# HuttleyLab/DiverseSeq

Measured on AMD Instinct MI355X. Metric: sequences scored/sec (delta-JSD, k=6), higher is better.
Workload: dtype f64 (results and every set update in f64; reject/accept decisions tiered: f32 and f32-log scores decide rows farther from the threshold than their proven error bands, f64 the rest)

## Files before the change

### diverseseq_amd/csrc/api.cpp

```cpp
#include "dvs_internal.h"

#include <cmath>
#include <cstring>
#include <mutex>

uint64_t dvs_pow_u64(uint32_t base, uint32_t exp, bool *overflow);
void dvs_matrix_free_fields(dvs_matrix *m);
int dvs_matrix_fill_counts(dvs_ctx *ctx, dvs_matrix *m, const dvs_seq_view &sv, const uint64_t *offsets, bool no_wait);
int dvs_matrix_fill_freq_entropy(dvs_ctx *ctx, dvs_matrix *m);
int dvs_hist_prepare(dvs_ctx *ctx, const uint64_t *offsets, uint32_t nseq, uint32_t k, uint64_t nbins, uint64_t nbytes, size_t *n_long_out);
bool dvs_hist_rows_fit_u16(const dvs_ctx *ctx, uint64_t B, size_t n_long);
int dvs_matrix_fill_freq_totals(dvs_ctx *ctx, dvs_matrix *m, const double *d_meta);
int dvs_matrix_fill_compacted(dvs_ctx *ctx, dvs_matrix *m, const double *d_in, const double *d_meta);

static std::string g_create_err;

int dvs_set_error(dvs_ctx *ctx, int code, const char *fmt, ...) {
    char buf[512];
    va_list ap;
    va_start(ap, fmt);
    vsnprintf(buf, sizeof buf, fmt, ap);
    va_end(ap);
    if (ctx) ctx->err = buf;
    else g_create_err = buf;
// ... 25 lines not shown
    if (e != hipSuccess) {
        *ptr = nullptr;
        return dvs_hip_fail(ctx, e, what);
    }
    ctx->live[*ptr] = sz;
    return DVS_OK;
}

void dvs_dev_free(dvs_ctx *ctx, void *ptr) {
    if (!ptr) return;
    auto it = ctx ? ctx->live.find(ptr) : std::map<void *, size_t>::iterator();
    if (!ctx || it == ctx->live.end()) {
        (void)hipFree(ptr);
        return;
    }
    ctx->pool.emplace(it->second, ptr);
    ctx->pool_bytes += it->second;
    ctx->live.erase(it);
}

int dvs_pinned_get(dvs_ctx *ctx, void **ptr) {
    if (!ctx->pinned_pool.empty()) {
        *ptr = ctx->pinned_pool.back();
        ctx->pinned_pool.pop_back();
        return DVS_OK;
    }
    hipError_t e = hipHostMalloc(ptr, 4096, hipHostMallocDefault);
    if (e != hipSuccess) return dvs_hip_fail(ctx, e, "hipHostMalloc");
    return DVS_OK;
}
void dvs_pinned_put(dvs_ctx *ctx, void *ptr) {
    if (!ptr) return;
    if (ctx) ctx->pinned_pool.push_back(ptr);
    else (void)hipHostFree(ptr);
}
hipEvent_t dvs_event_get(dvs_ctx *ctx) {
    if (!ctx->event_pool.empty()) {
        hipEvent_t e = ctx->event_pool.back();
        ctx->event_pool.pop_back();
        return e;
    }
    hipEvent_t e = nullptr;
    (void)hipEventCreate(&e);
    return e;
}
void dvs_event_put(dvs_ctx *ctx, hipEvent_t e) {
    if (!e) return;
    if (ctx) ctx->event_pool.push_back(e);
    else (void)hipEventDestroy(e);
}

void dvs_dev_trim(dvs_ctx *ctx) {
    (void)hipStreamSynchronize(ctx->stream);
    for (auto &kv : ctx->pool) (void)hipFree(kv.second);
    ctx->pool.clear();
    ctx->pool_bytes = 0;
}

void dvs_knobs_from_env(dvs_knobs *k) {
    auto on = [](const char *name) { return getenv(name) != nullptr; };
    *k = dvs_knobs();
    k->no_uniform_offsets = on("DVS_NO_UNIFORM_OFFSETS");
    k->no_offsets_cache = on("DVS_NO_OFFSETS_CACHE");
    k->counts_u32 = on("DVS_COUNTS_U32");
    k->build_wait = on("DVS_BUILD_WAIT");
    k->no_packed_upload = on("DVS_NO_PACKED_UPLOAD");
// ... 103 lines not shown
    const uint32_t words = uint32_t(ctx->n_cu + 31) / 32;
    std::vector<uint32_t> lo(words, 0u), hi(words, 0u);
    for (int i = 0; i < ctx->n_cu; i++) (i < head ? lo : hi)[i / 32] |= 1u << (i % 32);
    hipStream_t a = nullptr, b = nullptr;
    if (hipExtStreamCreateWithCUMask(&a, words, lo.data()) != hipSuccess ||
        hipExtStreamCreateWithCUMask(&b, words, hi.data()) != hipSuccess) {
        (void)hipGetLastError();
        if (a) (void)hipStreamDestroy(a);
        return false;
    }
    ctx->stream_head = a;
    ctx->stream_rest = b;
    ctx->head_cus = head;
    return true;
}

void dvs_ctx_retain(dvs_ctx *ctx) {
    if (ctx) ctx->refs++;
}

void dvs_ctx_release(dvs_ctx *ctx) {
    if (!ctx || --ctx->refs > 0) return;
    (void)hipSetDevice(ctx->device);
    dvs_dev_free(ctx, ctx->off_cache.d_off);
    dvs_dev_free(ctx, ctx->off_cache.d_rows);
    dvs_dev_free(ctx, ctx->off_cache.d_tiles);
    if (ctx->off_cache.ev_up) (void)hipEventDestroy(ctx->off_cache.ev_up);
    if (ctx->off_cache.h_off) (void)hipHostFree(ctx->off_cache.h_off);
    if (ctx->pack_ev) (void)hipEventDestroy(ctx->pack_ev);
    if (ctx->h_pack) (void)hipHostFree(ctx->h_pack);
    dvs_dev_free(ctx, ctx->d_clog_tbl);
    dvs_dev_trim(ctx);
    for (void *p : ctx->pinned_pool) (void)hipHostFree(p);
    for (hipEvent_t e : ctx->event_pool) (void)hipEventDestroy(e);
    if (ctx->stream2) (void)hipStreamDestroy(ctx->stream2);
    if (ctx->stream_head) (void)hipStreamDestroy(ctx->stream_head);
    if (ctx->stream_rest) (void)hipStreamDestroy(ctx->stream_rest);
    if (ctx->own_stream && ctx->stream) (void)hipStreamDestroy(ctx->stream);
    delete ctx;
}

extern "C" {

const char *dvs_last_error(const dvs_ctx *ctx) { return ctx ? ctx->err.c_str() : g_create_err.c_str(); }

int dvs_ctx_trim(dvs_ctx *ctx) {
    if (!ctx) return DVS_ERR_VALUE;
    dvs_dev_trim(ctx);
    return DVS_OK;
}

int dvs_ctx_sync(dvs_ctx *ctx) {
    if (!ctx) return DVS_ERR_VALUE;
    DVS_HIP(ctx, hipStreamSynchronize(ctx->stream));
    return DVS_OK;
}

int dvs_ctx_set_timing(dvs_ctx *ctx, int on) {
    if (!ctx) return DVS_ERR_VALUE;
    ctx->timing = on != 0;
    return DVS_OK;
}

int dvs_ctx_device_info(dvs_ctx *ctx, char *name, size_t name_len, int *n_cu, uint64_t *hbm_bytes) {
    if (!ctx) return DVS_ERR_VALUE;
    hipDeviceProp_t prop;
// ... 299 lines not shown
```

### diverseseq_amd/csrc/dvs_internal.h

```cpp
#pragma once

#include <hip/hip_runtime.h>

#include <cstdarg>
#include <cstdint>
#include <cstdio>
#include <functional>
#include <map>
#include <string>
#include <vector>

#include "../../include/dvs_hip.h"

#define DVS_EPS 2.220446049250313e-16
#define DVS_HEAD_ROWS 1024u

struct dvs_knobs {
    bool no_uniform_offsets = false;
    bool no_offsets_cache = false;
    bool counts_u32 = false;
    bool build_wait = false;
    bool no_packed_upload = false;
    bool cu_mask_set = false;
    bool no_fast_step = false;
    bool no_persist = false;
    bool no_head_phase = false;
    bool persist_no_seeded = false;
    bool persist_no_small = false;
    bool persist_no_coarse = false;
    bool persist_no_events = false;
    bool persist_debug = false;
    int persist_wg_rounds = -1;
    bool ingest_no_stream = false;
    bool test_persist_fake_error = false;
    uint32_t test_long_tile = 0;
    uint32_t test_rowlog_ring = 0;
};
void dvs_knobs_from_env(dvs_knobs *k);

struct dvs_ctx {
    dvs_knobs knobs;
    int device = 0;
    hipStream_t stream = nullptr;
    bool own_stream = false;
    hipStream_t stream2 = nullptr;
    hipStream_t stream_head = nullptr, stream_rest = nullptr;
    int head_cus = 0;
    bool cu_split_tried = false;
    int persist_timeouts = 0;
    int n_cu = 0;
    size_t lds_per_block = 0;
    double *d_clog_tbl = nullptr;
    bool timing = false;
    std::string err;
    std::multimap<size_t, void *> pool;
    std::vector<void *> pinned_pool;
    std::vector<hipEvent_t> event_pool;
    std::map<void *, size_t> live;
    size_t pool_bytes = 0;
    int refs = 1;
    bool owner_gone = false;
    std::map<const void *, size_t> lds_raised;
    std::map<std::pair<const void *, size_t>, bool> persist_fits;
    struct OffsetsCache {
        uint64_t *h_off = nullptr;
        size_t h_cap = 0, n_off = 0;
        hipEvent_t ev_up = nullptr;
        std::vector<uint32_t> h_long_rows;
        std::vector<unsigned char> h_tiles;
        uint64_t nbytes = 0;
        uint32_t k = 0;
        void *d_off = nullptr, *d_rows = nullptr, *d_tiles = nullptr;
        size_t d_off_cap = 0;
        size_t n_long = 0, n_tiles = 0;
        bool uniform = false;
        uint64_t uni_base = 0, uni_stride = 0;
    } off_cache;
    void *h_pack = nullptr;
    size_t h_pack_cap = 0;
    hipEvent_t pack_ev = nullptr;
};
int dvs_raise_dyn_lds(dvs_ctx *ctx, const void *fn, size_t bytes);
void dvs_ctx_retain(dvs_ctx *ctx);
hipStream_t dvs_ctx_stream2(dvs_ctx *ctx);
bool dvs_ctx_cu_split(dvs_ctx *ctx);
void dvs_ctx_release(dvs_ctx *ctx);

struct dvs_matrix;
int dvs_matrix_settle(dvs_ctx *ctx, const dvs_matrix *m);
int dvs_dev_alloc(dvs_ctx *ctx, void **ptr, size_t bytes, const char *what);
void dvs_dev_free(dvs_ctx *ctx, void *ptr);
void dvs_dev_trim(dvs_ctx *ctx);
struct PooledBuf {
    dvs_ctx *ctx;
    void *p = nullptr;
    ~PooledBuf() { dvs_dev_free(ctx, p); }
    template <typename T>
    T *as() { return static_cast<T *>(p); }
};
int dvs_pinned_get(dvs_ctx *ctx, void **ptr);
void dvs_pinned_put(dvs_ctx *ctx, void *ptr);
hipEvent_t dvs_event_get(dvs_ctx *ctx);
void dvs_event_put(dvs_ctx *ctx, hipEvent_t e);

int dvs_set_error(dvs_ctx *ctx, int code, const char *fmt, ...);
int dvs_hip_fail(dvs_ctx *ctx, hipError_t e, const char *what);

#define DVS_HIP(ctx, call)                                        \
    do {                                                          \
        hipError_t e__ = (call);                                  \
        if (e__ != hipSuccess) return dvs_hip_fail(ctx, e__, #call); \
    } while (0)

struct dvs_matrix {
    int kind = 0;
    uint16_t *d_counts16 = nullptr;
    uint32_t nrows = 0;
    uint64_t nbins = 0;
    uint32_t k = 0, num_states = 0;
    uint32_t *d_counts = nullptr;
    double *d_freqs = nullptr;
    uint32_t *d_totals = nullptr;
    double *d_entropy = nullptr;
    uint32_t *d_src_row = nullptr;
    std::vector<uint32_t> h_head_totals;
    uint32_t *h_head_pinned = nullptr;
    hipEvent_t ev_built = nullptr;
    hipEvent_t ev_join = nullptr;
    uint32_t head_count = 0;
    uint32_t head_rows_built = 0;
    bool rest_beside_head = false;
    int device = 0;
    dvs_ctx *ctx = nullptr;
};
// ... 135 lines not shown
```

### diverseseq_amd/csrc/persist.hip

```cpp
#include "select_dev.h"

#include <algorithm>
#include <type_traits>
#include <cstddef>
#include <cstdlib>
#include <cstring>

namespace {

constexpr int P_THREADS = 512;
constexpr int P_J = 8;
constexpr int P_CH = 16;
constexpr uint32_t P_MAXN = 512;
constexpr uint32_t P_MAXN_BIG = 256;
constexpr uint32_t P_MAXN_MAX = 896;
constexpr uint32_t p_maxn(bool cached, bool maxm = false) { return cached ? (maxm ? P_MAXN_MAX : P_MAXN) : P_MAXN_BIG; }
constexpr uint32_t P_SMALLN = 16;
constexpr uint32_t P_SMALL_ROWS = 13;
constexpr uint32_t p_maxjobs(bool cached, bool maxm = false) { return p_maxn(cached, maxm) + 1; }
constexpr size_t p_acc_bytes(uint32_t maxn) { return size_t(8) * (maxn + 1) * 2 * sizeof(unsigned long long); }
__device__ __forceinline__ unsigned long long p_acc_word(double v) {
    return ((unsigned long long)__double2ll_rn(v * 0x1p50) << 6) + 1ull;
}
__device__ __forceinline__ double p_acc_value(unsigned long long w) { return double((long long)w >> 6) * 0x1p-50; }
// ... 2810 lines not shown
            const unsigned long long d1 = p_acc_complete(acc + uint64_t(tid) * 2 + 1, s_prev + tid * 2 + 1, HO_K, acc_ok);
            unsigned long long e0 = 0ull, e1 = 0ull;
            for (uint32_t q = 0; q < HO_K; q++) {
                const uint32_t h2 = ho_hash(epoch, tid * HO_K + q);
                e0 += p_acc_word(double((h2 >> 4) & 0xFFFFu) * (1.0 / 65536.0));
                e1 += p_acc_word(double(h2 & 0xFFu) * (1.0 / 4096.0));
            }
            acc_wrong = !acc_ok || d0 != e0 || d1 != e1;
        }
        if (__syncthreads_or(acc_wrong ? 1 : 0) && tid == 0) fails++;
        if (mirror && epoch + 1 < rounds) {
            if (tid == 0) __hip_atomic_store(&sync->wrec[(epoch + 1) & 1u][b], p_word(epoch + 1, SEL_NONE, false), RLX_AGENT);
            early_rec = epoch + 1;
            for (uint32_t z = (h >> 16) & 15u; z > 0; z--) __builtin_amdgcn_s_sleep(16);
        }
    }
    if (tid == 0 && fails) atomicAdd(bad, fails);
    if (tid == 0 && __hip_atomic_load(&sync->timeout, RLX_AGENT)) atomicAdd(bad, 1ull << 32);
}

}

template <typename T>
static const void *persist_fn(const dvs_select *s) {
    const bool cached = s->dev.B <= uint64_t(P_J) * P_THREADS;
    if (s->params.mode == DVS_MODE_MAX) return reinterpret_cast<const void *>(persist_nmost_kernel<T, true, true>);
    if constexpr (std::is_same_v<T, uint16_t>) {
        if (s->persist_small) return reinterpret_cast<const void *>(persist_nmost_kernel<T, true, false, true>);
    }
    return cached ? reinterpret_cast<const void *>(persist_nmost_kernel<T, true>)
                  : reinterpret_cast<const void *>(persist_nmost_kernel<T, false>);
}

static int persist_prepare(dvs_ctx *ctx, dvs_select *s, uint32_t head_stop, hipStream_t on) {
    std::vector<unsigned char> &image = head_stop ? s->h_psync_head : s->h_psync;
    image.assign(sizeof(PSync), 0);
    PSync &init = *reinterpret_cast<PSync *>(image.data());
    init.stop_at = head_stop;
    init.seeded = s->persist_seeded ? 1u : 0u;
    init.seed_list = static_cast<const unsigned long long *>(s->d_seed_list);
    for (int g = 0; g < 8; g++) init.rel[g].hint = ~0ull;
    init.wg_thresh = s->params.window ? 0u : 4u;
    init.wg_scale = 1.5f;
    if (ctx->knobs.persist_wg_rounds >= 0) init.wg_thresh = uint32_t(ctx->knobs.persist_wg_rounds);
    init.no_coarse = (ctx->knobs.persist_no_coarse ? 1u : 0u) | (ctx->knobs.persist_no_events ? 2u : 0u) |
                     0u;
    init.small_rows = s->persist_small ? s->persist_small_rows : 0u;
    init.lds_bytes = uint32_t(s->persist_lds);
    init.wmax = uint32_t(std::min<uint64_t>(s->npos, 0xFFFFFFFFull));
    DVS_HIP(ctx, hipMemcpyAsync(head_stop ? s->psync_head : s->psync, &init, sizeof init, hipMemcpyHostToDevice, on));
    DVS_HIP(ctx, hipMemsetAsync(head_stop ? s->ppart_head : s->ppart, 0, p_acc_bytes(s->persist_maxn), on));
    return DVS_OK;
}

template <typename T>
static int persist_launch(dvs_ctx *ctx, dvs_select *s, const T *mat, uint32_t grid, uint32_t head_stop,
                          hipStream_t on) {
    const SelDev &d = s->dev;
    if (head_stop ? !s->head_prepared : !s->persist_prepared) {
        int prc = persist_prepare(ctx, s, head_stop, on);
        if (prc) return prc;
    }
    if (head_stop) s->head_prepared = false;
    else s->persist_prepared = false;
    s->persist_seeded = false;
    const hipEvent_t e1 = dvs_scan_timing_start(ctx, s, on);
    const void *fn = persist_fn<T>(s);
    SelDev d_arg = d;
    const T *mat_arg = mat;
    PSync *sync_arg = static_cast<PSync *>(head_stop ? s->psync_head : s->psync);
    unsigned long long *part_arg = static_cast<unsigned long long *>(head_stop ? s->ppart_head : s->ppart);
    uint32_t g_arg = grid;
    void *args[] = {&d_arg, &mat_arg, &sync_arg, &part_arg, &g_arg};
    hipError_t le = hipLaunchKernel(fn, dim3(grid), dim3(P_THREADS), args, s->persist_lds, on);
    if (s->time_scan) (void)hipEventRecord(e1, on);
    if (le != hipSuccess) {
        (void)hipGetLastError();
        return DVS_ERR_UNSUPPORTED;
    }
    DVS_HIP(ctx, hipGetLastError());
    return DVS_OK;
}

int dvs_persist_setup(dvs_ctx *ctx, dvs_select *s) {
// ... 17 lines not shown
               size_t(maxn_ + 1) * 16 +
               (maxm ? p_batch_lds() : 0);
    };
    size_t lds = lds_for(p_maxn(cached, maxm));
    if (s->persist_small) {
        const size_t lds_small = lds_for(P_SMALLN) + size_t(s->persist_small_rows) * B * 2 + 16;
        if (lds_small <= ctx->lds_per_block) lds = lds_small;
        else s->persist_small = false;
    }
    if (cached && !maxm && s->mat_kind != 1 && !s->persist_small)
        lds += size_t(p_maxn(cached, maxm)) * 4 + size_t(P_J) * P_THREADS * (s->mat_kind == 2 ? 2 : 4);
    s->persist_maxn = s->persist_small ? P_SMALLN : p_maxn(cached, maxm);
    s->persist_maxjobs = s->persist_small ? P_SMALLN + 1 : p_maxjobs(cached, maxm);
    if (!maxm && s->cap > s->persist_maxn) return DVS_OK;
    if (lds > ctx->lds_per_block) return DVS_OK;
    s->persist_lds = lds;
    const void *fn = dvs_mat_dispatch(s->mat, [&](auto *mp) -> const void * {
        using T = std::remove_cv_t<std::remove_pointer_t<decltype(mp)>>;
        return persist_fn<T>(s);
    });
    int rc = dvs_raise_dyn_lds(ctx, fn, lds);
    if (rc) return rc;
    {
        auto key = std::make_pair(fn, lds);
        auto hit = ctx->persist_fits.find(key);
        if (hit == ctx->persist_fits.end()) {
            int per_cu = 0;
            const bool fits = hipOccupancyMaxActiveBlocksPerMultiprocessor(&per_cu, fn, P_THREADS, lds) == hipSuccess && per_cu >= 1;
            if (!fits) (void)hipGetLastError();
            hit = ctx->persist_fits.emplace(key, fits).first;
        }
        if (!hit->second) return DVS_OK;
    }
    rc = dvs_dev_alloc(ctx, &s->psync, sizeof(PSync), "persistent sync block");
    if (!rc) rc = dvs_dev_alloc(ctx, &s->ppart, p_acc_bytes(s->persist_maxn) + (maxm ? 2 * p_batch_bytes() : 0),
                                "leave-one-out accumulators");
    if (rc) return rc;
    s->persist = true;
    return DVS_OK;
}

#ifdef DVS_PERSIST_STAMPS
static void persist_trace_report(const void *blk, uint32_t G) {
    std::vector<unsigned long long> tr(4 * 8 * 256);
    if (hipMemcpy(tr.data(), static_cast<const char *>(blk) + offsetof(PSync, trace), tr.size() * 8, hipMemcpyDeviceToHost) != hipSuccess) return;
    for (int w_ = 0; w_ < 4; w_++) {
        const unsigned long long *t0 = &tr[(w_ * 8 + 0) * 256], *t1 = &tr[(w_ * 8 + 1) * 256], *t2 = &tr[(w_ * 8 + 2) * 256], *tg = &tr[(w_ * 8 + 3) * 256];
        const unsigned long long *t4 = &tr[(w_ * 8 + 4) * 256], *t5 = &tr[(w_ * 8 + 5) * 256], *t6 = &tr[(w_ * 8 + 6) * 256], *t7 = &tr[(w_ * 8 + 7) * 256];
        if (!tg[2] || G < 4) continue;
        std::vector<double> top, arr, seen, pub, tot, end_;
        unsigned long long first_top = ~0ull;
        for (uint32_t b = 0; b + 2 < G; b++) if (t0[b]) first_top = std::min(first_top, t0[b]);
        for (uint32_t b = 0; b + 2 < G; b++) {
            if (!t0[b] || !t1[b] || !t2[b]) continue;
            top.push_back((t0[b] - first_top) / 100.0);
            arr.push_back((t1[b] - first_top) / 100.0);
            seen.push_back((double(t2[b]) - double(tg[2])) / 100.0);
            if (t4[b] > tg[2] && t5[b] > tg[2] && t6[b] > tg[2]) {
                pub.push_back((double(t4[b]) - double(tg[2])) / 100.0);
                tot.push_back((double(t5[b]) - double(tg[2])) / 100.0);
                end_.push_back((double(t6[b]) - double(tg[2])) / 100.0);
            }
        }
        if (arr.empty()) continue;
        auto srt = [](std::vector<double> &v) { std::sort(v.begin(), v.end()); };
        srt(top); srt(arr); srt(seen);
        auto q_ = [](const std::vector<double> &v, double f) { return v[size_t(f * (v.size() - 1))]; };
        fprintf(stderr, "[dvs persist trace] window %d: tops 0 / %.2f / %.2f (min/median/max us), records stored %.2f / %.2f / %.2f / %.2f (min/median/90%%/max), "
                "gather begun %.2f, last record seen %.2f, release stored %.2f, release seen +%.2f / +%.2f / +%.2f (min/median/max after it was stored)\n",
                w_ * 12 + 12, q_(top, 0.5), top.back(), arr.front(), q_(arr, 0.5), q_(arr, 0.9), arr.back(),
// ... 48 lines not shown
        for (int w = 0; w < 2; w++)
            fprintf(stderr, "[dvs persist %s] us: scan %.1f bar1 %.1f resolve %.1f loo %.1f bar2 %.1f | partials %.1f combine %.1f lowest-row fetch %.1f rebuild %.1f\n",
                    w ? "mirror block" : "block 0", dbg[0 + 16 * w] / 100.0, dbg[1 + 16 * w] / 100.0,
                    dbg[2 + 16 * w] / 100.0, dbg[3 + 16 * w] / 100.0, dbg[4 + 16 * w] / 100.0,
                    dbg[6 + 16 * w] / 100.0, dbg[7 + 16 * w] / 100.0, dbg[8 + 16 * w] / 100.0,
                    dbg[5 + 16 * w] / 100.0);
#ifdef DVS_PERSIST_STAMPS
        persist_trace_report(blk, which ? s->persist_grid : uint32_t(ctx->head_cus));
#endif
        if (dbg[15] + dbg[14])
            fprintf(stderr, "[dvs persist block 0] accepts for which its leave-one-out job was ready when the release came: %llu (the candidate's frequencies: %llu)\n", dbg[15], dbg[14]);
        if (dbg[9] + dbg[10] + dbg[11] + dbg[12])
            fprintf(stderr, "[dvs persist block 0] us inside the phases: window top %.1f own rows scanned %.1f hint look + record %.1f (then: scan = the rest) | behind the rebuild %.1f\n",
                    dbg[9] / 100.0, dbg[10] / 100.0, dbg[11] / 100.0, dbg[12] / 100.0);
        if (dbg[16 + 10] + dbg[16 + 12])
            fprintf(stderr, "[dvs persist] scan + rendezvous: row-per-workgroup windows %llu (%.1f us, %llu rows), "
                    "row-per-wave windows %llu (%.1f us, %llu rows)\n", dbg[16 + 10], dbg[16 + 9] / 100.0,
                    dbg[16 + 13], dbg[16 + 12], dbg[16 + 11] / 100.0, dbg[16 + 14]);
    }
}

void dvs_persist_debug_done(const SelCtl &c) {
    fprintf(stderr, "[dvs persist] launches ended early: replica full %u, sum check %u, push argmin %u, stat comparison %u, "
            "candidate in band %u, replace argmin %u, state not taken %u / %u\n", c.why[0], c.why[1], c.why[2], c.why[3],
            c.why[4], c.why[5], c.why[6], c.why[7]);
}

int dvs_persist_launch(dvs_ctx *ctx, dvs_select *s) {
    return dvs_mat_dispatch(s->mat, [&](auto *mp) { return persist_launch(ctx, s, mp, s->persist_grid, 0u, ctx->stream); });
}

static int persist_head_blocks(dvs_ctx *ctx, dvs_select *s) {
    if (s->psync_head) return DVS_OK;
    int rc = dvs_dev_alloc(ctx, &s->psync_head, sizeof(PSync), "head phase sync block");
    if (!rc) rc = dvs_dev_alloc(ctx, &s->ppart_head, p_acc_bytes(s->persist_maxn), "head phase accumulators");
    return rc;
}

int dvs_persist_launch_head(dvs_ctx *ctx, dvs_select *s, uint32_t grid, uint32_t stop_at, hipStream_t on) {
    int rc = persist_head_blocks(ctx, s);
    if (rc) return rc;
    return dvs_mat_dispatch(s->mat, [&](auto *mp) { return persist_launch(ctx, s, mp, grid, stop_at, on); });
}

int dvs_persist_prepare_head(dvs_ctx *ctx, dvs_select *s, uint32_t stop_at, hipStream_t on) {
    int rc = persist_head_blocks(ctx, s);
    if (!rc) rc = persist_prepare(ctx, s, stop_at, on);
    if (!rc) s->head_prepared = true;
    return rc;
}

int dvs_persist_prepare_main(dvs_ctx *ctx, dvs_select *s) {
    int rc = persist_prepare(ctx, s, 0u, ctx->stream);
    if (!rc) s->persist_prepared = true;
    return rc;
}

extern "C" int dvs_selftest_handover(dvs_ctx *ctx, uint32_t rounds, uint64_t *failures) {
    if (!ctx || !failures || !rounds) return dvs_set_error(ctx, DVS_ERR_VALUE, "bad argument");
    if (rounds >= P_EPOCH_MAX) return dvs_set_error(ctx, DVS_ERR_VALUE, "at most %u rounds", P_EPOCH_MAX - 1);
    DVS_HIP(ctx, hipSetDevice(ctx->device));
    const uint32_t G = uint32_t(std::min(ctx->n_cu, int(P_MAXG)));
    if (G < HO_MEMBERS * HO_K + 2 || ctx->knobs.cu_mask_set)
        return dvs_set_error(ctx, DVS_ERR_UNSUPPORTED, "the self-test wants %u co-resident workgroups", HO_MEMBERS * HO_K + 2);
    void *d_sync = nullptr, *d_acc = nullptr, *d_bad = nullptr;
    int rc = dvs_dev_alloc(ctx, &d_sync, sizeof(PSync), "self-test sync block");
    if (!rc) rc = dvs_dev_alloc(ctx, &d_acc, p_acc_bytes(HO_MEMBERS), "self-test accumulators");
    if (!rc) rc = dvs_dev_alloc(ctx, &d_bad, 8, "self-test counter");
// ... 25 lines not shown
```

### diverseseq_amd/csrc/select.h

```cpp
#pragma once

#include "dvs_internal.h"

#define SEL_NONE 0xFFFFFFFFFFFFFFFFull
#define SEL_SEEDS_AT 512

enum : uint32_t { SEL_RUN = 0, SEL_DONE = 1, SEL_ARBITER = 2, SEL_ERROR = 3,
                  SEL_NEED_SETUP = 4 };
enum : uint32_t { ARB_RESOLVE = 1, ARB_FINALIZE = 2 };
enum : uint32_t { FORCE_NONE = 0, FORCE_ACCEPT = 1, FORCE_REJECT = 2, FORCE_COMMIT = 3, FORCE_ROLLBACK = 4 };

struct SelCtl {
    unsigned long long cursor;
    unsigned long long npos;
    unsigned long long event_pos;
    unsigned long long arb_pos;
    unsigned long long rows_scored, rows_rechecked;
    unsigned long long rows_coarse_passed;
    unsigned long long rows_before_launch;
    uint32_t window, window_min, window_max;
    uint32_t status, arb_stage, forced, forced_lowest;
    uint32_t size, lowest, mode, max_size, stat;
    uint32_t ev_kind;
    uint32_t ev_n;
// ... 37 lines not shown
    uint8_t *inset = nullptr;
    uint32_t *wg_rows = nullptr;
    unsigned long long *evlog_pos = nullptr;
    uint32_t *evlog_kind = nullptr;
    const double *gather_all = nullptr;
    uint32_t gather_world = 0;
    double *rowlog = nullptr;
    uint32_t rowlog_cap = 0;
};

struct dvs_select {
    dvs_ctx *ctx = nullptr;
    dvs_select_params params{};
    const dvs_matrix *mat = nullptr;
    int mat_kind = 0;
    uint64_t npos = 0;
    uint32_t cap = 0;
    SelDev dev;
    SelCtl *h_ctl = nullptr;
    SelCtl ctl0{};
    std::vector<uint32_t> h_order, h_labels;
    std::vector<uint32_t> h_out_labels;
    std::vector<uint64_t> seed_positions;
    uint32_t scan_grid = 0, loo_grid = 0;
    size_t scan_lds = 0;
    bool base_in_lds = true;
    bool scan_hot = false;
    bool persist = false;
    uint32_t persist_grid = 0, persist_maxn = 0, persist_maxjobs = 0;
    bool persist_small = false;
    uint32_t persist_small_rows = 0;
    size_t persist_lds = 0;
    void *psync = nullptr;
    std::vector<unsigned char> h_psync;
    std::vector<unsigned char> h_psync_head;
    void *ppart = nullptr;
    double *d_mbres = nullptr;
    uint32_t mb_jw = 0;
    uint32_t mb_launched = 0;
    void *psync_head = nullptr, *ppart_head = nullptr;
    bool persist_seeded = false;
    bool seeded_start = false;
    bool head_prepared = false;
    bool persist_prepared = false;
    bool used_side_streams = false;
    hipEvent_t ev_side_done = nullptr;
    void *d_seed_list = nullptr;
    bool seed_list_in_ctl = false;
    bool inset_clean = false;
    hipStream_t setup_side = nullptr;
    bool head_phase = false;
    int batch = 16;
    bool time_scan = false;
    std::vector<hipEvent_t> ev_pool;
    size_t ev_used = 0;
    double scan_ms = 0.0;
    double scan_ms_last = 0.0;
    uint64_t scan_launches = 0;
    uint32_t n_arbitrated = 0;
    double arbiter_ms = 0.0;
    bool fast_step = false;
    bool fs_need_scan = false;
    unsigned long long *h_fshist = nullptr;
    unsigned long long fs_launches = 0;
    unsigned long long fs_peek_floor = 0;
    double *fs_slot = nullptr;
    double *fs_packed = nullptr;
    double *d_jobres = nullptr;
    void *d_fsync = nullptr;
    uint32_t fs_K = 1, fs_jobs = 0, fs_grid = 0;
    size_t fs_lds = 0;
    std::vector<double> h_rowlog;
    uint64_t rowlog_have = 0;
    uint32_t steps_since_poll = 0;
    void *arbiter = nullptr;
};

int dvs_select_arbitrate(dvs_ctx *ctx, dvs_select *s);
// ... 12 lines not shown
```

### diverseseq_amd/csrc/select.hip

```cpp
#include "dvs_internal.h"
#include "select.h"
#include "select_dev.h"

#include <algorithm>
#include <chrono>
#include <type_traits>
#include <cmath>
#include <cstring>
#include <cstdlib>
#include <memory>

namespace {

constexpr int SCAN_THREADS = 512;
constexpr int WIDE_THREADS = 1024;
constexpr int LOO_THREADS = 256;

template <typename T>
__device__ __forceinline__ void scan_rows_hot(SelCtl *ctl, const T *__restrict__ mat,
                                              const uint32_t *__restrict__ totals,
                                              const double *__restrict__ rowH, const double *bvec,
                                              uint64_t B, const ScanState &st, uint64_t first,
                                              uint64_t stride, uint32_t lane, uint32_t &nread,
                                              uint32_t &nprecise) {
// ... 1718 lines not shown
}

__global__ __launch_bounds__(LOO_THREADS) void gather_members_kernel(SelDev d, double *__restrict__ rows,
                                                                    double *__restrict__ meta) {
    const uint32_t r = blockIdx.x, n = d.ctl->size;
    double *out = rows + uint64_t(r) * d.B;
    if (r >= n) {
        for (uint64_t i = threadIdx.x; i < d.B; i += LOO_THREADS) out[i] = 0.0;
        if (threadIdx.x == 0) meta[2 * r] = meta[2 * r + 1] = 0.0;
        return;
    }
    const uint32_t slot = d.ord[r];
    const double *src = d.M + uint64_t(slot) * d.B;
    for (uint64_t i = threadIdx.x; i < d.B; i += LOO_THREADS) out[i] = src[i];
    if (threadIdx.x == 0) {
        meta[2 * r] = double(d.mPos[slot]);
        meta[2 * r + 1] = 1.0;
    }
}

template <typename T>
__global__ __launch_bounds__(LOO_THREADS) void pack_event_kernel(SelDev d, const T *__restrict__ mat,
                                                                double *__restrict__ slot) {
    pack_event_body<T>(d, mat, slot);
}

}

static void sel_free(dvs_select *s) {
    if (!s) return;
#ifdef DVS_FS_TRACE
    fs_trace_report(s);
#endif
    if (s->used_side_streams && s->ctx) {
        if (s->ctx->stream_head) (void)hipStreamSynchronize(s->ctx->stream_head);
        if (s->ctx->stream2) (void)hipStreamSynchronize(s->ctx->stream2);
    }
    void *ptrs[] = {s->dev.ctl, s->dev.S, s->dev.Stmp, s->dev.base, s->dev.cand, s->dev.M,
                    s->dev.mH, s->dev.mDelta, s->dev.dtmp, s->dev.dsum, s->dev.mLabel, s->dev.mPos,
                    s->dev.ord, s->dev.inset, s->dev.wg_rows, s->dev.evlog_pos, s->dev.evlog_kind, s->dev.rowlog,
                    (void *)s->dev.order, (void *)s->dev.labels};
    for (void *p : ptrs)
        dvs_dev_free(s->ctx, p);
    if (s->fs_launches && s->ctx) (void)hipStreamSynchronize(s->ctx->stream);
    dvs_pinned_put(s->ctx, s->h_ctl);
    dvs_pinned_put(s->ctx, s->h_fshist);
    for (hipEvent_t e : s->ev_pool) dvs_event_put(s->ctx, e);
    dvs_dev_free(s->ctx, s->d_mbres);
    dvs_dev_free(s->ctx, s->d_jobres);
    dvs_dev_free(s->ctx, s->d_fsync);
    dvs_dev_free(s->ctx, s->psync);
    dvs_dev_free(s->ctx, s->ppart);
    dvs_dev_free(s->ctx, s->psync_head);
    dvs_dev_free(s->ctx, s->ppart_head);
    if (!s->seed_list_in_ctl) dvs_dev_free(s->ctx, s->d_seed_list);
    if (s->ev_side_done) dvs_event_put(s->ctx, s->ev_side_done);
    dvs_select_arbiter_free(s);
    dvs_ctx_release(s->ctx);
    delete s;
}

hipEvent_t dvs_scan_timing_start(dvs_ctx *ctx, dvs_select *s, hipStream_t on) {
    if (!s->time_scan) return nullptr;
    if (s->ev_used + 2 > s->ev_pool.size()) {
        hipEvent_t a = dvs_event_get(ctx), b = dvs_event_get(ctx);
        s->ev_pool.push_back(a);
        s->ev_pool.push_back(b);
    }
    s->ev_used += 2;
    (void)hipEventRecord(s->ev_pool[s->ev_used - 2], on);
    return s->ev_pool[s->ev_used - 1];
}

static void sel_add_scan_times(dvs_select *s) {
    for (size_t i = 0; i + 1 < s->ev_used; i += 2) {
        float ms = 0.f;
        if (hipEventElapsedTime(&ms, s->ev_pool[i], s->ev_pool[i + 1]) == hipSuccess) {
            s->scan_ms += ms;
            s->scan_ms_last = ms;
        }
        s->scan_launches++;
    }
    s->ev_used = 0;
}

template <typename T>
static void launch_scan(const dvs_select *s, const T *mat, bool hot, SelCtl *ctl, uint32_t *wg_rows, hipStream_t st) {
// ... 10 lines not shown
static void launch_iteration(dvs_ctx *ctx, dvs_select *s, const T *mat, int stage, hipStream_t on = nullptr) {
    const SelDev &d = s->dev;
    const hipStream_t stream = on ? on : ctx->stream;
    if (stage == 0) {
        const hipEvent_t e1 = dvs_scan_timing_start(ctx, s, stream);
        launch_scan<T>(s, mat, s->scan_hot, d.ctl, d.wg_rows, stream);
        if (s->time_scan) (void)hipEventRecord(e1, stream);
    }
    if (stage <= 1)
        hipLaunchKernelGGL((resolve_kernel<T>), dim3(1), dim3(WIDE_THREADS), 0, stream, d, mat);
    hipLaunchKernelGGL(loo_kernel, dim3(s->loo_grid + 1), dim3(LOO_THREADS), 0, stream, d, s->scan_grid);
    hipLaunchKernelGGL(finalize_kernel, dim3(1), dim3(WIDE_THREADS), 0, stream, d);
}

template <typename T>
static int launch_max_batch(dvs_ctx *ctx, dvs_select *s, const T *mat, uint32_t size_bound) {
    if (!s->d_mbres) {
        s->mb_jw = std::min<uint32_t>(s->cap, MB_MAX_MEMBERS) + 3;
        int rc = dvs_dev_alloc(ctx, (void **)&s->d_mbres, size_t(3) * MB_ROWS * s->mb_jw * sizeof(double), "max batch results");
        if (rc) return rc;
    }
    if (size_bound + 3 > s->mb_jw) return DVS_OK;
    hipLaunchKernelGGL((max_batch_jobs_kernel<T>), dim3(size_bound + 3, MB_ROWS / MB_RG), dim3(MB_THREADS), 0, ctx->stream, s->dev, mat,
                       s->d_mbres, s->mb_jw);
    hipLaunchKernelGGL(max_batch_decide_kernel, dim3(1), dim3(WIDE_THREADS), 0, ctx->stream, s->dev, s->d_mbres, s->mb_jw);
    s->mb_launched++;
    return DVS_OK;
}

static int sel_poll(dvs_ctx *ctx, dvs_select *s) {
    DVS_HIP(ctx, hipMemcpyAsync(s->h_ctl, s->dev.ctl, sizeof(SelCtl), hipMemcpyDeviceToHost,
                                ctx->stream));
    DVS_HIP(ctx, hipStreamSynchronize(ctx->stream));
    return DVS_OK;
}

template <typename T>
static int sel_seed(dvs_ctx *ctx, dvs_select *s, const T *mat, hipStream_t st, bool light = false);

template <typename T>
static int sel_drop_seeded(dvs_ctx *ctx, dvs_select *s, const T *mat, hipStream_t st) {
    s->seeded_start = false;
    s->persist_seeded = false;
    return sel_seed<T>(ctx, s, mat, st);
}

template <typename T>
static int sel_leave_persist(dvs_ctx *ctx, dvs_select *s, const T *mat, bool restart) {
    s->persist = false;
    if (!restart) return DVS_OK;
    dvs_select_arbiter_free(s);
    return sel_drop_seeded<T>(ctx, s, mat, ctx->stream);
}

template <typename T>
static int sel_arbitrate(dvs_ctx *ctx, dvs_select *s, const T *mat) {
    const SelCtl &c = *s->h_ctl;
    if (s->params.flags & DVS_SELECT_NO_ARBITER)
        return dvs_set_error(ctx, DVS_ERR_UNSUPPORTED,
                             "ambiguous decision at stream position %llu (stage %u): "
                             "|score - threshold| within the rounding band",
                             (unsigned long long)c.arb_pos, c.arb_stage);
    const uint32_t stage = c.arb_stage;
    const auto t_arb = std::chrono::steady_clock::now();
    const int rc = dvs_select_arbitrate(ctx, s);
    s->arbiter_ms += std::chrono::duration<double, std::milli>(std::chrono::steady_clock::now() - t_arb).count();
// ... 99 lines not shown
    s->setup_side = nullptr;
    s->head_phase = false;
    if (s->mat->head_rows_built && s->params.n_seed <= s->mat->head_rows_built && s->h_order.empty() &&
        !(s->params.flags & DVS_SELECT_STEPWISE)) {
        s->head_phase = s->mat->rest_beside_head && ctx->stream_head && s->persist &&
                        s->params.mode == DVS_MODE_NMOST && s->params.window == 0 &&
                        s->cap + 2 <= uint32_t(ctx->head_cus) && s->npos > 4ull * s->mat->head_rows_built &&
                        s->params.n_seed + 64 <= s->mat->head_rows_built && !ctx->knobs.no_head_phase;
        s->setup_side = s->head_phase ? ctx->stream_head : dvs_ctx_stream2(ctx);
    }
}

template <typename T>
static int sel_start(dvs_ctx *ctx, dvs_select *s, const T *mat) {
    hipStream_t side = s->setup_side;
    const bool head_phase = s->head_phase;
    hipStream_t st = side ? side : ctx->stream;
    if (side) s->used_side_streams = true;
    int rc = sel_seed<T>(ctx, s, mat, st, s->seeded_start);
    if (rc) return rc;
    if (head_phase) {
        rc = dvs_persist_launch_head(ctx, s, uint32_t(ctx->head_cus), s->mat->head_rows_built, side);
        if (rc == DVS_ERR_UNSUPPORTED)
            rc = s->seeded_start ? sel_drop_seeded<T>(ctx, s, mat, st) : DVS_OK;
        if (rc) return rc;
        rc = dvs_persist_prepare_main(ctx, s);
        if (rc) return rc;
        const_cast<dvs_matrix *>(s->mat)->rest_beside_head = false;
    }
    if (side) {
        if (!s->ev_side_done) s->ev_side_done = dvs_event_get(ctx);
        DVS_HIP(ctx, hipEventRecord(s->ev_side_done, side));
        DVS_HIP(ctx, hipStreamWaitEvent(ctx->stream, s->ev_side_done, 0));
    }
    if (s->params.flags & DVS_SELECT_STEPWISE) return sel_poll(ctx, s);
    return sel_run_loop<T>(ctx, s, mat);
}

template <typename T>
static int sel_seed(dvs_ctx *ctx, dvs_select *s, const T *mat, hipStream_t st, bool light) {
    const std::vector<uint64_t> &seeds = s->seed_positions;
    SelDev &d = s->dev;
    SelCtl c = s->ctl0;
    const uint32_t wdef = s->params.window ? s->params.window : (s->persist ? s->persist_grid * 2u : 4096u);
    c.window_min = wdef;
    c.window_max = std::max<uint32_t>(wdef, s->scan_grid * (SCAN_THREADS / 64) * 8);
    c.window = wdef;
    *s->h_ctl = c;
    if (!s->inset_clean || st != (s->setup_side ? s->setup_side : ctx->stream))
        DVS_HIP(ctx, hipMemsetAsync(d.inset, 0, std::max<size_t>(d.nlabels, 1), st));
    s->inset_clean = false;
    if (!s->d_seed_list) {
        int rc0 = dvs_dev_alloc(ctx, &s->d_seed_list, seeds.size() * sizeof(uint64_t), "seed list");
        if (rc0) return rc0;
    }
    uint64_t *d_seed = static_cast<uint64_t *>(s->d_seed_list);
    if (s->seed_list_in_ctl) {
        std::memcpy(reinterpret_cast<unsigned char *>(s->h_ctl) + SEL_SEEDS_AT, seeds.data(), seeds.size() * sizeof(uint64_t));
        DVS_HIP(ctx, hipMemcpyAsync(d.ctl, s->h_ctl, SEL_SEEDS_AT + seeds.size() * sizeof(uint64_t), hipMemcpyHostToDevice, st));
    } else {
        DVS_HIP(ctx, hipMemcpyAsync(d.ctl, s->h_ctl, sizeof c, hipMemcpyHostToDevice, st));
        DVS_HIP(ctx, hipMemcpyAsync(d_seed, seeds.data(), seeds.size() * sizeof(uint64_t),
                                    hipMemcpyHostToDevice, st));
    }
    if (light) {
        DVS_HIP(ctx, hipGetLastError());
// ... 157 lines not shown
        DVS_HIP(ctx, hipMemcpyAsync((void *)d.order, order, size_t(npos) * 4, hipMemcpyHostToDevice, ctx->stream));
    }
    if (labels) {
        if (int rc = dvs_dev_alloc(ctx, (void **)&d.labels, size_t(npos) * 4, "d.labels")) return rc;
        DVS_HIP(ctx, hipMemcpyAsync((void *)d.labels, labels, size_t(npos) * 4, hipMemcpyHostToDevice, ctx->stream));
    }
    static_assert(sizeof(SelCtl) <= 4096, "control block must fit a cached pinned block");
    return dvs_pinned_get(ctx, (void **)&s->h_ctl);
}

static int sel_prepare_engine(dvs_ctx *ctx, dvs_select *s, const uint32_t *order, const uint32_t *labels) {
    SelDev &d = s->dev;
    const dvs_matrix *m = s->mat;
    const uint32_t n_seed = s->params.n_seed, nlabels = d.nlabels;
    int rc = dvs_persist_setup(ctx, s);
    if (rc) return rc;
    sel_plan_setup_stream(ctx, s);
    if (s->setup_side) s->used_side_streams = true;
    DVS_HIP(ctx, hipMemsetAsync(d.inset, 0, std::max<size_t>(nlabels, 1), s->setup_side ? s->setup_side : ctx->stream));
    s->inset_clean = true;
    DVS_HIP(ctx, hipMemsetAsync(d.wg_rows, 0, size_t(s->scan_grid) * 8, s->setup_side ? s->setup_side : ctx->stream));
    s->seeded_start = s->persist && s->params.mode == DVS_MODE_NMOST && d.B <= 4096 && !order && !labels &&
                      !(s->params.flags & DVS_SELECT_STEPWISE) && n_seed >= 2 && n_seed <= 32 && !ctx->knobs.persist_no_seeded;
    s->persist_seeded = s->seeded_start;
    if (size_t(n_seed) * sizeof(uint64_t) <= 4096 - SEL_SEEDS_AT) {
        s->d_seed_list = reinterpret_cast<unsigned char *>(d.ctl) + SEL_SEEDS_AT;
        s->seed_list_in_ctl = true;
    } else if (s->seeded_start) {
        if ((rc = dvs_dev_alloc(ctx, &s->d_seed_list, size_t(n_seed) * sizeof(uint64_t), "seed list"))) return rc;
    }
    if (s->persist && m->rest_beside_head && ctx->stream_head && m->head_rows_built && s->params.mode == DVS_MODE_NMOST &&
        !order && !labels) {
        s->used_side_streams = true;
        return dvs_persist_prepare_head(ctx, s, m->head_rows_built, ctx->stream_head);
    }
    return DVS_OK;
}

static int sel_read_seeds(dvs_ctx *ctx, dvs_select *s, const uint32_t *order) {
    const dvs_matrix *m = s->mat;
    const uint32_t n_seed = s->params.n_seed;
    std::vector<uint32_t> h_tot(n_seed);
    int rc = dvs_matrix_settle(ctx, m);
    if (rc) return rc;
    hipError_t ce = hipSuccess;
    if (!order && n_seed && n_seed <= m->h_head_totals.size()) {
        std::copy(m->h_head_totals.begin(), m->h_head_totals.begin() + n_seed, h_tot.begin());
    } else if (!order && n_seed) {
        ce = hipMemcpyAsync(h_tot.data(), m->d_totals, size_t(n_seed) * 4, hipMemcpyDeviceToHost, ctx->stream);
    } else {
        for (uint64_t p = 0; p < n_seed && ce == hipSuccess; p++)
            ce = hipMemcpyAsync(&h_tot[p], m->d_totals + order[p], 4, hipMemcpyDeviceToHost, ctx->stream);
    }
    if ((order || n_seed > m->h_head_totals.size()) &&
        (hipStreamSynchronize(ctx->stream) != hipSuccess || ce != hipSuccess))
        return dvs_set_error(ctx, DVS_ERR_RUNTIME, "reading the seed rows' totals failed");
    std::vector<uint64_t> &seeds = s->seed_positions;
    for (uint64_t p = 0; p < n_seed; p++)
        if (h_tot[p] > 0) seeds.push_back(p);
    if (seeds.size() < 2)
        return seeds.empty() ? dvs_set_error(ctx, DVS_ERR_VALUE, "records cannot be empty")
                             : dvs_set_error(ctx, DVS_ERR_VALUE, "must have > 1 KmerSeq");
    return DVS_OK;
}

static void sel_init_ctl(dvs_ctx *ctx, dvs_select *s) {
// ... 463 lines not shown
```

Before: 69.56 million.

## Upload persist sync image and zeroed accumulators in one pinned copy

The persistent sync block and its leave-one-out accumulators now share one device allocation, and the host image is a pooled pinned buffer. A single host-to-device copy then initializes both when the image fits in 32 KB, replacing a pageable memcpy plus a memset. Teardown also skips redundant side-stream synchronizations once the side streams are known to have been joined before the final control readback. This adds in-flight tracking for the pinned images, a larger host-to-device transfer of zeros, and more complex teardown ordering logic.

```diff
diff --git a/diverseseq_amd/csrc/api.cpp b/diverseseq_amd/csrc/api.cpp
--- a/diverseseq_amd/csrc/api.cpp
+++ b/diverseseq_amd/csrc/api.cpp
@@ -81,6 +81,23 @@
 void dvs_pinned_put(dvs_ctx *ctx, void *ptr) {
     if (!ptr) return;
     if (ctx) ctx->pinned_pool.push_back(ptr);
+    else (void)hipHostFree(ptr);
+}
+int dvs_pinned_get_sized(dvs_ctx *ctx, size_t bytes, void **ptr) {
+    const size_t sz = ((bytes ? bytes : 1) + 4095) & ~size_t(4095);
+    auto it = ctx->pinned_sized.find(sz);
+    if (it != ctx->pinned_sized.end()) {
+        *ptr = it->second;
+        ctx->pinned_sized.erase(it);
+        return DVS_OK;
+    }
+    hipError_t e = hipHostMalloc(ptr, sz, hipHostMallocDefault);
+    if (e != hipSuccess) return dvs_hip_fail(ctx, e, "hipHostMalloc");
+    return DVS_OK;
+}
+void dvs_pinned_put_sized(dvs_ctx *ctx, void *ptr, size_t bytes) {
+    if (!ptr) return;
+    if (ctx) ctx->pinned_sized.emplace(((bytes ? bytes : 1) + 4095) & ~size_t(4095), ptr);
     else (void)hipHostFree(ptr);
 }
 hipEvent_t dvs_event_get(dvs_ctx *ctx) {
@@ -250,6 +267,7 @@
     dvs_dev_free(ctx, ctx->d_clog_tbl);
     dvs_dev_trim(ctx);
     for (void *p : ctx->pinned_pool) (void)hipHostFree(p);
+    for (auto &kv : ctx->pinned_sized) (void)hipHostFree(kv.second);
     for (hipEvent_t e : ctx->event_pool) (void)hipEventDestroy(e);
     if (ctx->stream2) (void)hipStreamDestroy(ctx->stream2);
     if (ctx->stream_head) (void)hipStreamDestroy(ctx->stream_head);
diff --git a/diverseseq_amd/csrc/dvs_internal.h b/diverseseq_amd/csrc/dvs_internal.h
--- a/diverseseq_amd/csrc/dvs_internal.h
+++ b/diverseseq_amd/csrc/dvs_internal.h
@@ -55,6 +55,7 @@
     std::string err;
     std::multimap<size_t, void *> pool;
     std::vector<void *> pinned_pool;
+    std::multimap<size_t, void *> pinned_sized;
     std::vector<hipEvent_t> event_pool;
     std::map<void *, size_t> live;
     size_t pool_bytes = 0;
@@ -100,6 +101,8 @@
 };
 int dvs_pinned_get(dvs_ctx *ctx, void **ptr);
 void dvs_pinned_put(dvs_ctx *ctx, void *ptr);
+int dvs_pinned_get_sized(dvs_ctx *ctx, size_t bytes, void **ptr);
+void dvs_pinned_put_sized(dvs_ctx *ctx, void *ptr, size_t bytes);
 hipEvent_t dvs_event_get(dvs_ctx *ctx);
 void dvs_event_put(dvs_ctx *ctx, hipEvent_t e);
 
diff --git a/diverseseq_amd/csrc/persist.hip b/diverseseq_amd/csrc/persist.hip
--- a/diverseseq_amd/csrc/persist.hip
+++ b/diverseseq_amd/csrc/persist.hip
@@ -2866,10 +2866,22 @@
                   : reinterpret_cast<const void *>(persist_nmost_kernel<T, false>);
 }
 
+constexpr size_t P_ACC_AT = (sizeof(PSync) + 255) & ~size_t(255);
+constexpr size_t P_IMAGE_MAX = 32 * 1024;
+static size_t p_image_bytes(uint32_t maxn) {
+    return P_ACC_AT + p_acc_bytes(maxn) <= P_IMAGE_MAX ? P_ACC_AT + p_acc_bytes(maxn) : sizeof(PSync);
+}
+
 static int persist_prepare(dvs_ctx *ctx, dvs_select *s, uint32_t head_stop, hipStream_t on) {
-    std::vector<unsigned char> &image = head_stop ? s->h_psync_head : s->h_psync;
-    image.assign(sizeof(PSync), 0);
-    PSync &init = *reinterpret_cast<PSync *>(image.data());
+    void *&image = head_stop ? s->h_psync_head : s->h_psync;
+    s->psync_image_bytes = p_image_bytes(s->persist_maxn);
+    if (head_stop ? s->head_image_in_flight : s->image_in_flight) DVS_HIP(ctx, hipStreamSynchronize(on));
+    if (!image) {
+        int rc = dvs_pinned_get_sized(ctx, s->psync_image_bytes, &image);
+        if (rc) return rc;
+    }
+    std::memset(image, 0, s->psync_image_bytes);
+    PSync &init = *static_cast<PSync *>(image);
     init.stop_at = head_stop;
     init.seeded = s->persist_seeded ? 1u : 0u;
     init.seed_list = static_cast<const unsigned long long *>(s->d_seed_list);
@@ -2882,8 +2894,10 @@
     init.small_rows = s->persist_small ? s->persist_small_rows : 0u;
     init.lds_bytes = uint32_t(s->persist_lds);
     init.wmax = uint32_t(std::min<uint64_t>(s->npos, 0xFFFFFFFFull));
-    DVS_HIP(ctx, hipMemcpyAsync(head_stop ? s->psync_head : s->psync, &init, sizeof init, hipMemcpyHostToDevice, on));
-    DVS_HIP(ctx, hipMemsetAsync(head_stop ? s->ppart_head : s->ppart, 0, p_acc_bytes(s->persist_maxn), on));
+    (head_stop ? s->head_image_in_flight : s->image_in_flight) = true;
+    DVS_HIP(ctx, hipMemcpyAsync(head_stop ? s->psync_head : s->psync, image, s->psync_image_bytes, hipMemcpyHostToDevice, on));
+    if (s->psync_image_bytes < P_ACC_AT + p_acc_bytes(s->persist_maxn))
+        DVS_HIP(ctx, hipMemsetAsync(head_stop ? s->ppart_head : s->ppart, 0, p_acc_bytes(s->persist_maxn), on));
     return DVS_OK;
 }
 
@@ -2967,10 +2981,10 @@
         }
         if (!hit->second) return DVS_OK;
     }
-    rc = dvs_dev_alloc(ctx, &s->psync, sizeof(PSync), "persistent sync block");
-    if (!rc) rc = dvs_dev_alloc(ctx, &s->ppart, p_acc_bytes(s->persist_maxn) + (maxm ? 2 * p_batch_bytes() : 0),
-                                "leave-one-out accumulators");
+    rc = dvs_dev_alloc(ctx, &s->psync, P_ACC_AT + p_acc_bytes(s->persist_maxn) + (maxm ? 2 * p_batch_bytes() : 0),
+                       "persistent sync block + leave-one-out accumulators");
     if (rc) return rc;
+    s->ppart = static_cast<unsigned char *>(s->psync) + P_ACC_AT;
     s->persist = true;
     return DVS_OK;
 }
@@ -3085,8 +3099,8 @@
 
 static int persist_head_blocks(dvs_ctx *ctx, dvs_select *s) {
     if (s->psync_head) return DVS_OK;
-    int rc = dvs_dev_alloc(ctx, &s->psync_head, sizeof(PSync), "head phase sync block");
-    if (!rc) rc = dvs_dev_alloc(ctx, &s->ppart_head, p_acc_bytes(s->persist_maxn), "head phase accumulators");
+    int rc = dvs_dev_alloc(ctx, &s->psync_head, P_ACC_AT + p_acc_bytes(s->persist_maxn), "head phase sync block + accumulators");
+    if (!rc) s->ppart_head = static_cast<unsigned char *>(s->psync_head) + P_ACC_AT;
     return rc;
 }
 
diff --git a/diverseseq_amd/csrc/select.h b/diverseseq_amd/csrc/select.h
--- a/diverseseq_amd/csrc/select.h
+++ b/diverseseq_amd/csrc/select.h
@@ -93,8 +93,10 @@
     uint32_t persist_small_rows = 0;
     size_t persist_lds = 0;
     void *psync = nullptr;
-    std::vector<unsigned char> h_psync;
-    std::vector<unsigned char> h_psync_head;
+    void *h_psync = nullptr, *h_psync_head = nullptr;
+    size_t psync_image_bytes = 0;
+    bool image_in_flight = false;
+    bool head_image_in_flight = false;
     void *ppart = nullptr;
     double *d_mbres = nullptr;
     uint32_t mb_jw = 0;
@@ -105,6 +107,9 @@
     bool head_prepared = false;
     bool persist_prepared = false;
     bool used_side_streams = false;
+    bool side_work_elsewhere = false;
+    bool side_join_queued = false;
+    bool side_streams_joined = false;
     hipEvent_t ev_side_done = nullptr;
     void *d_seed_list = nullptr;
     bool seed_list_in_ctl = false;
diff --git a/diverseseq_amd/csrc/select.hip b/diverseseq_amd/csrc/select.hip
--- a/diverseseq_amd/csrc/select.hip
+++ b/diverseseq_amd/csrc/select.hip
@@ -1774,7 +1774,7 @@
 #ifdef DVS_FS_TRACE
     fs_trace_report(s);
 #endif
-    if (s->used_side_streams && s->ctx) {
+    if (s->used_side_streams && !s->side_streams_joined && s->ctx) {
         if (s->ctx->stream_head) (void)hipStreamSynchronize(s->ctx->stream_head);
         if (s->ctx->stream2) (void)hipStreamSynchronize(s->ctx->stream2);
     }
@@ -1784,7 +1784,9 @@
                     (void *)s->dev.order, (void *)s->dev.labels};
     for (void *p : ptrs)
         dvs_dev_free(s->ctx, p);
-    if (s->fs_launches && s->ctx) (void)hipStreamSynchronize(s->ctx->stream);
+    if ((s->fs_launches || s->image_in_flight) && s->ctx) (void)hipStreamSynchronize(s->ctx->stream);
+    dvs_pinned_put_sized(s->ctx, s->h_psync, s->psync_image_bytes);
+    dvs_pinned_put_sized(s->ctx, s->h_psync_head, s->psync_image_bytes);
     dvs_pinned_put(s->ctx, s->h_ctl);
     dvs_pinned_put(s->ctx, s->h_fshist);
     for (hipEvent_t e : s->ev_pool) dvs_event_put(s->ctx, e);
@@ -1792,9 +1794,7 @@
     dvs_dev_free(s->ctx, s->d_jobres);
     dvs_dev_free(s->ctx, s->d_fsync);
     dvs_dev_free(s->ctx, s->psync);
-    dvs_dev_free(s->ctx, s->ppart);
     dvs_dev_free(s->ctx, s->psync_head);
-    dvs_dev_free(s->ctx, s->ppart_head);
     if (!s->seed_list_in_ctl) dvs_dev_free(s->ctx, s->d_seed_list);
     if (s->ev_side_done) dvs_event_put(s->ctx, s->ev_side_done);
     dvs_select_arbiter_free(s);
@@ -1871,6 +1871,9 @@
     DVS_HIP(ctx, hipMemcpyAsync(s->h_ctl, s->dev.ctl, sizeof(SelCtl), hipMemcpyDeviceToHost,
                                 ctx->stream));
     DVS_HIP(ctx, hipStreamSynchronize(ctx->stream));
+    s->side_streams_joined = s->side_join_queued;
+    s->image_in_flight = false;
+    if (s->side_streams_joined) s->head_image_in_flight = false;
     return DVS_OK;
 }
 
@@ -2036,6 +2039,7 @@
         if (!s->ev_side_done) s->ev_side_done = dvs_event_get(ctx);
         DVS_HIP(ctx, hipEventRecord(s->ev_side_done, side));
         DVS_HIP(ctx, hipStreamWaitEvent(ctx->stream, s->ev_side_done, 0));
+        s->side_join_queued = !s->side_work_elsewhere;
     }
     if (s->params.flags & DVS_SELECT_STEPWISE) return sel_poll(ctx, s);
     return sel_run_loop<T>(ctx, s, mat);
@@ -2259,6 +2263,7 @@
     if (s->persist && m->rest_beside_head && ctx->stream_head && m->head_rows_built && s->params.mode == DVS_MODE_NMOST &&
         !order && !labels) {
         s->used_side_streams = true;
+        if (s->setup_side != ctx->stream_head) s->side_work_elsewhere = true;
         return dvs_persist_prepare_head(ctx, s, m->head_rows_built, ctx->stream_head);
     }
     return DVS_OK;
```

New measurement: 70.64 million (median of 6 runs). 1.6% higher.
